# yanivw12/gs2mesh

Hardware: AMD Instinct MI355X
Metric: stereo-pair renders/sec + TSDF Mvoxel-updates/sec (higher is better)
Workload: dtype f32

## Files before the change

gs2mesh_amd/_lib.py:

```python
from __future__ import annotations

import ctypes as C

import numpy as np
import os

_HERE = os.path.dirname(os.path.abspath(__file__))
LIB_PATH = os.path.join(_HERE, "libgs2mesh_amd.so")

vp = C.c_void_p
i32 = C.c_int
i64 = C.c_int64
f32 = C.c_float
f64 = C.c_double


class Camera(C.Structure):
    _fields_ = [("width", C.c_int32), ("height", C.c_int32), ("tanfovx", f32), ("tanfovy", f32),
                ("viewmatrix", f32 * 16), ("projmatrix", f32 * 16), ("campos", f32 * 3)]


class Gaussians(C.Structure):
    _fields_ = [("P", C.c_int32), ("sh_degree", C.c_int32), ("M", C.c_int32), ("raw", C.c_int32),
                ("xyz", vp), ("scales", vp), ("rotations", vp), ("opacities", vp), ("shs", vp), ("shs_rest", vp)]
# ... 7 lines not shown
OPT_BIN_WORKGROUPS = 9
OPT_BIN_WG_THREADS = 10
OPT_BLEND_MODE = 11
TSDF_MAP_HEADER_BYTES = 32
OPT_BLEND_PROFILE = 12
OPT_BIN_LANE_TILES = 13
OPT_PROJECT_SHARED_READ = 14
BLEND_PROF_COUNTERS = ("waves", "wave_cycles", "dma_wait", "staging", "prefetch_issue", "loop", "epilogue", "batches",
                       "staged_instances", "listed_instances")
XFORM_SUM_F32, XFORM_RAW_F32, XFORM_SUM_PACKED = 0, 1, 2
XFORM_PACKED_MAX_FRAMES = 1023
OPT_DEBUG_SYNC = 3
OPT_STAGE_TIMING = 4
RASTER_STAGES = ("project", "hist_colscan", "tile_scan", "scatter", "sort_tiles", "blend", "count_tiles")
TSDF_STAGES = ("tsdf_touch", "tsdf_integrate")

_PROTOS = {
    "gs2m_version": (i32, []),
    "gs2m_last_error": (C.c_char_p, []),
    "gs2m_raster_create": (i32, [C.POINTER(vp), i32]),
    "gs2m_raster_destroy": (i32, [vp]),
    "gs2m_raster_set_option": (i32, [vp, i32, i32]),
    "gs2m_raster_reserve": (i32, [vp, i32, i32, i32, i32, i64]),
    "gs2m_rasterize_forward": (i32, [vp, i32, i32, i32, vp, i32, i32, vp, vp, vp, vp, vp, f32, vp, vp, vp, vp, vp,
                                     f32, f32, i32, vp, vp, i32, vp]),
    "gs2m_mark_visible": (i32, [i32, vp, vp, vp, vp, vp]),
    "gs2m_render_views": (i32, [vp, C.POINTER(Gaussians), C.POINTER(Camera), i32, C.POINTER(f32), f32, vp, vp, vp,
                                vp]),
    "gs2m_raster_pack_sh": (i32, [vp, C.POINTER(Gaussians), vp]),
    "gs2m_raster_pack_model": (i32, [vp, C.POINTER(Gaussians), vp, vp]),
    "gs2m_raster_pack_invalidate": (i32, [vp]),
    "gs2m_raster_status": (i32, [vp, vp, i32, C.POINTER(i64), C.POINTER(i32), C.POINTER(i64)]),
    "gs2m_raster_stage_times": (i32, [vp, vp, C.POINTER(f64), C.POINTER(i64)]),
    "gs2m_raster_blend_cycles": (i32, [vp, vp, C.POINTER(C.c_uint64)]),
    "gs2m_raster_download_geometry": (i32, [vp, vp, i32, i32, vp, vp, vp, vp, vp, vp]),
    "gs2m_raster_download_binning": (i32, [vp, vp, i32, i64, vp, C.c_int32, vp]),
    "gs2m_tsdf_extract_count": (i32, [vp, vp, C.POINTER(i64)]),
    "gs2m_tsdf_extract": (i32, [vp, vp, i64, vp, vp, C.POINTER(i64)]),
    "gs2m_tsdf_extract_indexed": (i32, [vp, vp, i64, vp, vp, vp, C.POINTER(i64)]),
    "gs2m_stereo_depth_occlusion": (i32, [vp, vp, i32, i32, f64, f64, vp, vp, vp]),
    "gs2m_mask_preprocess": (i32, [i32, i32, i32, C.POINTER(vp), C.POINTER(vp), i32, i32, i32, i32, C.POINTER(vp), vp, vp]),
    "gs2m_tsdf_create": (i32, [C.POINTER(vp), f64, f64, i32, i32, i32, i64, i32]),
    "gs2m_tsdf_destroy": (i32, [vp]),
    "gs2m_tsdf_reset": (i32, [vp, vp]),
    "gs2m_tsdf_integrate": (i32, [vp, vp, vp, vp, i32, i32, f64, f64, f64, f64, C.POINTER(f64), f64, f64, f64, vp]),
    "gs2m_tsdf_integrate_batch": (i32, [vp, i32, C.POINTER(vp), C.POINTER(vp), C.POINTER(vp), i32, i32, f64, f64, f64, f64,
                                        C.POINTER(f64), f64, f64, f64, vp]),
    "gs2m_tsdf_set_stage_timing": (i32, [vp, i32]),
    "gs2m_tsdf_stage_times": (i32, [vp, vp, C.POINTER(f64), C.POINTER(i64)]),
# ... 118 lines not shown
```

gs2mesh_amd/csrc/raster_api.hip:

```cpp
#include <stdarg.h>
#include <stdio.h>
#include <stdlib.h>
#include <string.h>

#include <string>
#include <vector>

#include "../../include/gs2mesh_amd.h"
#include "raster_internal.h"
#include "roctx_ranges.h"

static thread_local std::string g_err;
void gs2m_set_error(const char* fmt, ...) {
    char buf[1024];
    va_list ap;
    va_start(ap, fmt);
    vsnprintf(buf, sizeof(buf), fmt, ap);
    va_end(ap);
    g_err = buf;
}
extern "C" const char* gs2m_last_error(void) { return g_err.c_str(); }
extern "C" int gs2m_version(void) { return GS2M_VERSION; }

#define HIPCHK(expr)                                                                          \
    do {                                                                                      \
        hipError_t e__ = (expr);                                                              \
        if (e__ != hipSuccess) {                                                              \
            gs2m_set_error("%s failed: %s (%s:%d)", #expr, hipGetErrorString(e__), __FILE__, __LINE__); \
            return 1;                                                                         \
        }                                                                                     \
    } while (0)

#define GS2M_SORT_CLASSES_API 3
#define GS2M_MAX_STATUS 64

struct gs2m_raster {
    int device = 0;
    int opt_exact_cull = 0, opt_blend = 4, opt_debug = 0, opt_timing = 0, opt_tile_rows = 1, opt_pair_batch = 0;
    int opt_bin_workgroups = 256, opt_bin_wg_threads = 1024, opt_blend_mode = 2;
    int opt_blend_profile = 0;
    int opt_project_shared = 0;
    int opt_bin_lane_tiles = 4;
    unsigned long long* d_blend_prof = nullptr;
    struct EvPair {
        int stage;
        hipEvent_t a, b;
    };
    std::vector<EvPair> ev_live;
    std::vector<hipEvent_t> ev_free;
// ... 3 lines not shown
    unsigned long long* d_tilemask = nullptr;
    float* d_shpack = nullptr;
    size_t shpack_cap = 0;
    const float* pack_src = nullptr;
    const float* pack_src_rest = nullptr;
    int pack_P = 0;
    float* d_pk_xyz = nullptr;
    float* d_pk_scales = nullptr;
    float* d_pk_rots = nullptr;
    float* d_pk_opac = nullptr;
    int* d_order = nullptr;
    int* d_rank = nullptr;
    size_t pk_cap3 = 0, pk_cap3s = 0, pk_cap4 = 0, pk_cap1 = 0, order_cap = 0, rank_cap = 0;
    const float* model_src[4] = {nullptr, nullptr, nullptr, nullptr};
    bool model_packed = false;
    bool hint_valid = false;
    bool last_packed = false;
    const int* run_rank = nullptr;
    size_t mask_cap = 0;
    unsigned* d_hist = nullptr;
    size_t hist_cap = 0;
    unsigned* d_tile_count = nullptr;
    unsigned* d_tile_start = nullptr;
    size_t tile_cap = 0;
    unsigned* d_sort_lists = nullptr;
    size_t sort_lists_cap = 0;
    unsigned long long* d_keys = nullptr;
    unsigned long long* d_tmp = nullptr;
    size_t keys_cap_total = 0;
    unsigned inst_cap = 0;
    ViewStatus* d_status = nullptr;
// ... 45 lines not shown
    (void)hipFree(r->d_shpack);
    (void)hipFree(r->d_pk_xyz);
    (void)hipFree(r->d_pk_scales);
    (void)hipFree(r->d_pk_rots);
    (void)hipFree(r->d_pk_opac);
    (void)hipFree(r->d_order);
    (void)hipFree(r->d_rank);
    (void)hipFree(r->d_hist);
    (void)hipFree(r->d_tile_count);
    (void)hipFree(r->d_tile_start);
    (void)hipFree(r->d_sort_lists);
    (void)hipFree(r->d_keys);
    (void)hipFree(r->d_tmp);
    (void)hipFree(r->d_status);
    (void)hipFree(r->d_blend_prof);
    (void)hipHostFree(r->h_status);
    for (auto& p : r->ev_live) {
        (void)hipEventDestroy(p.a);
        (void)hipEventDestroy(p.b);
    }
    for (auto e : r->ev_free) (void)hipEventDestroy(e);
    delete r;
    return 0;
}

extern "C" int gs2m_raster_set_option(gs2m_raster* r, int option, int value) {
    if (!r) {
        gs2m_set_error("null handle");
        return 1;
    }
// ... 153 lines not shown
    StageTimer(gs2m_raster* r_, hipStream_t st_, int stage_) : r(r_), st(st_), stage(stage_), range(kStageRange[stage_]) {
        if (r->opt_timing) {
            a = ev_get(r);
            b = ev_get(r);
            if (a) (void)hipEventRecord(a, st);
        }
    }
    ~StageTimer() {
        if (a && b) {
            (void)hipEventRecord(b, st);
            r->ev_live.push_back({stage, a, b});
        }
    }
};

static int run_views(gs2m_raster* r, const GaussIn& g, int nv, int pairs, int W, int H, float* out_color,
                     unsigned char* out_rgb8, int* out_radii, int status_slot, hipStream_t st, const CamUniform* host_cams) {
    const int nvt = nv * pairs;
    const int gx = (W + GS2M_TILE - 1) / GS2M_TILE, gy = (H + GS2M_TILE - 1) / GS2M_TILE;
    const int gys = (gy + r->opt_tile_rows - 1) / r->opt_tile_rows;
    const int tiles = gx * gys;
    int hint[3] = {-1, -1, -1};
    int interleave = 1;
    if (r->hint_valid && r->last_tiles == tiles && r->last_nv == nvt) {
        unsigned nr_max = 0;
        for (int c = 0; c < 3; ++c) {
            unsigned m = 0;
            for (int v = 0; v < nvt; ++v) {
                const unsigned x = r->h_status[1 + status_slot + v].n_class[c];
                m = x > m ? x : m;
            }
            hint[c] = m > 0x3fffffffu ? -1 : (int)m;
        }
        for (int v = 0; v < nvt; ++v) {
            const unsigned x = r->h_status[1 + status_slot + v].num_rendered;
            nr_max = x > nr_max ? x : nr_max;
        }
        if (nr_max > 0u && nr_max <= 0x3fffffffu) interleave = (size_t)nr_max >= (size_t)800 * (size_t)tiles;
    }
    int chunk, n_wg;
    geometry(r, g.P, &chunk, &n_wg, pairs);
    int wg_threads = (gs2m_count_threads(chunk, r->opt_bin_wg_threads) + 63) / 64 * 64;
    while (wg_threads > 64 && (gs2m_scatter_lds_bytes(nv, tiles, wg_threads) > 160 * 1024 || gs2m_count_lds_bytes(nv, tiles, wg_threads) > 160 * 1024))
        wg_threads = (wg_threads / 2 + 63) / 64 * 64;
    const size_t lds = gs2m_scatter_lds_bytes(nv, tiles, wg_threads);
    const size_t lds_p = gs2m_count_lds_bytes(nv, tiles, wg_threads);
    if (lds > 160 * 1024 || lds_p > 160 * 1024) {
        gs2m_set_error("image %dx%d: %d views x %d tiles do not fit the 160 KiB LDS tile cursors", W, H, nv, tiles);
        return 1;
    }
    if (r->inst_cap == 0) {
        int64_t guess = (int64_t)g.P * 4;
// ... 21 lines not shown
        gs2m_launch_hist_colscan(st, nvt, r->d_hist, n_wg, tiles, r->d_tile_count);
    }
    if (dbg_check(r, st, "hist_colscan")) return 1;
    {
        StageTimer tm(r, st, GS2M_STAGE_TILESCAN);
        gs2m_launch_tile_scan(st, nvt, r->d_tile_count, r->d_tile_start, tiles, gx, r->h_status + 1 + status_slot, r->d_status, cap, r->d_sort_lists);
    }
    if (dbg_check(r, st, "tile_scan")) return 1;
    {
        StageTimer tm(r, st, GS2M_STAGE_SCATTER);
        if (gs2m_launch_scatter(nv, pairs, n_wg, wg_threads, lds, st, recs, g.P, r->d_cams, chunk, r->d_hist, r->d_tile_start,
                                r->d_tilemask, r->d_keys, cap, cull_arg_s, g.ids, g.ids != nullptr, r->opt_bin_lane_tiles))
            return 1;
    }
    if (dbg_check(r, st, "scatter")) return 1;
    {
        StageTimer tm(r, st, GS2M_STAGE_SORT);
        gs2m_launch_sort_tiles(st, nvt, r->d_keys, r->d_tmp, r->d_tile_start, tiles, cap, r->d_sort_lists, hint);
    }
    if (dbg_check(r, st, "sort_tiles")) return 1;
    {
        StageTimer tm(r, st, GS2M_STAGE_BLEND);
        if (gs2m_launch_blend(st, r->opt_blend, r->opt_tile_rows, nvt, gx, gy, r->d_keys, r->d_tile_start, recs, r->d_cams,
                              g.P, cap, out_color, out_rgb8, g.ids ? r->run_rank : nullptr,
                              r->d_sort_lists + (size_t)nvt * GS2M_SORT_CLASSES_API * (tiles + 1), r->opt_blend_mode,
                              r->opt_blend_profile ? r->d_blend_prof : nullptr, interleave))
            return 1;
    }
    if (dbg_check(r, st, "blend")) return 1;
    r->last_P = g.P;
    r->hint_valid = true;
    r->last_packed = g.ids != nullptr;
    r->last_nv = nvt;
    r->last_tiles = tiles;
    r->last_cap = cap;
    return 0;
}

extern "C" int gs2m_rasterize_forward(gs2m_raster* r, int P, int D, int M, const float* background, int width,
                                      int height, const float* means3D, const float* shs,
                                      const float* colors_precomp, const float* opacities, const float* scales,
                                      float scale_modifier, const float* rotations, const float* cov3D_precomp,
                                      const float* viewmatrix, const float* projmatrix, const float* cam_pos,
                                      float tan_fovx, float tan_fovy, int prefiltered, float* out_color,
                                      int* radii, int debug, gs2m_stream stream) {
    (void)prefiltered;
    if (!r) {
        gs2m_set_error("null handle");
        return 1;
    }
// ... 161 lines not shown
            u.gy = (H + GS2M_TILE - 1) / GS2M_TILE;
            u.bg[0] = bg[0];
            u.bg[1] = bg[1];
            u.bg[2] = bg[2];
            u.th = 16 * r->opt_tile_rows;
        }
        if (run_views(r, g, nv, pairs, W, H, out_color ? out_color + 3 * img * v0 : nullptr,
                      out_rgb8 ? out_rgb8 + 3 * img * v0 : nullptr,
                      out_radii ? out_radii + (size_t)gs->P * v0 : nullptr, v0, st, cu))
            return 1;
        v0 += nvt;
    }
    return 0;
}

static int pack_common(gs2m_raster* r, const gs2m_gaussians* gs, const int32_t* order, gs2m_stream stream, const char* who) {
    if (!r || !gs) {
        gs2m_set_error("%s: NULL argument", who);
        return 1;
    }
    r->pack_src = nullptr;
    r->pack_src_rest = nullptr;
    r->pack_P = 0;
    r->model_packed = false;
    if (gs->P <= 0 || gs->M != 16 || !gs->shs) return 0;
    HIPCHK(hipSetDevice(r->device));
    hipStream_t st = (hipStream_t)stream;
    const size_t P = (size_t)gs->P;
    const size_t groups = (P + 63) / 64;
    if (ensure(&r->d_shpack, &r->shpack_cap, groups * 12 * 64 * 4)) return 1;
// ... 227 lines not shown
```

gs2mesh_amd/csrc/raster_bin.hip:

```cpp
#include "raster_sort.h"
#include "raster_internal.h"

void gs2m_launch_hist_colscan(hipStream_t st, int nv, unsigned* hist, int n_wg, int tiles, unsigned* tile_count) {
    GS2M_LAUNCH(k_hist_colscan, dim3((tiles + 63) / 64, nv), dim3(64 * GS2M_COLSCAN_SEGS), 0, st, hist, n_wg, tiles, tile_count);
}
void gs2m_launch_tile_scan(hipStream_t st, int nv, const unsigned* tile_count, unsigned* tile_start, int tiles, int gx,
                           ViewStatus* status, ViewStatus* sticky, unsigned cap, unsigned* sort_lists) {
    GS2M_LAUNCH(k_tile_scan, dim3(nv), dim3(1024), 0, st, tile_count, tile_start, tiles, gx, status, sticky, cap, sort_lists);
}
size_t gs2m_sort_lists_words(int nv, int tiles) { return (size_t)nv * (GS2M_SORT_CLASSES * (tiles + 1) + tiles); }
void gs2m_launch_sort_tiles(hipStream_t st, int nv, unsigned long long* keys, unsigned long long* tmp,
                            const unsigned* tile_start, int tiles, unsigned cap, const unsigned* sort_lists, const int* class_hint) {
    const int fold = class_hint && class_hint[0] == 0 && class_hint[1] == 0 && class_hint[2] == 0;
    GS2M_LAUNCH(k_sort_tiles_small<4>, dim3((tiles + 3) / 4, nv), dim3(256), 0, st, keys, tile_start, tiles, cap, tmp, sort_lists, fold);
    if (fold) return;
    const int full[3] = {tiles < 1024 ? tiles : 1024, tiles < 512 ? tiles : 512, tiles < 512 ? tiles : 512};
    int g[3];
    for (int c = 0; c < 3; ++c) {
        g[c] = full[c];
        if (class_hint && class_hint[c] >= 0) {
            const int want = class_hint[c] + class_hint[c] / 2 + 16;
            g[c] = want < full[c] ? want : full[c];
        }
        if (g[c] < 1) g[c] = 1;
    }
    GS2M_LAUNCH(k_sort_tiles_bucket_4096x8, dim3(g[0], nv), dim3(512), 0, st, keys, tile_start, tiles, cap, sort_lists);
    GS2M_LAUNCH(k_sort_tiles_bucket_8192x8, dim3(g[1], nv), dim3(1024), 0, st, keys, tile_start, tiles, cap, sort_lists);
    GS2M_LAUNCH(k_sort_tiles, dim3(g[2], nv), dim3(256), 0, st, keys, tmp, tile_start, tiles, cap, sort_lists);
}
```

gs2mesh_amd/csrc/raster_internal.h:

```cpp
#pragma once
#include "raster_common.h"

size_t gs2m_scatter_lds_bytes(int nv, int tiles, int threads);
void gs2m_launch_project(int nv, int pairs, hipStream_t st, const GaussIn& g, CamUniform* cams, GeomRecs recs, int* radii,
                         int exact_cull, const CamUniform* host_cams, int shared_read);
int gs2m_launch_count_tiles(int nv, int pairs, int n_wg, int threads, size_t lds_bytes, hipStream_t st, GeomRecs recs, int P,
                            const CamUniform* cams, int chunk, unsigned* hist, unsigned long long* tilemask,
                            int exact_cull, int interleave, int lane_tiles);
int gs2m_count_threads(int chunk, int max_threads);
size_t gs2m_count_lds_bytes(int nv, int tiles, int threads);
int gs2m_launch_scatter(int nv, int pairs, int n_wg, int threads, size_t lds_bytes, hipStream_t st, GeomRecs recs, int P,
                        const CamUniform* cams, int chunk, const unsigned* hist, const unsigned* tile_start,
                        const unsigned long long* tilemask, unsigned long long* keys, unsigned cap, int exact_cull,
                        const int* ids, int interleave, int lane_tiles);
void gs2m_launch_pack_sh(hipStream_t st, int P, const float* shs, const float* shs_rest, float* packed, const int* order);
void gs2m_launch_pack_model(hipStream_t st, int P, const int* order, const float* xyz, const float* scales, const float* rots,
                            const float* opac, float* p_xyz, float* p_scales, float* p_rots, float* p_opac, int* rank,
                            unsigned* bad);
void gs2m_launch_mark_visible(hipStream_t st, int P, const float* xyz, const float* viewmatrix,
                              unsigned char* present);
void gs2m_launch_pack_camera(hipStream_t st, CamUniform* cams, int slot, const float* viewmatrix,
                             const float* projmatrix, const float* campos, const float* bg, float tanfovx,
                             float tanfovy, int W, int H, int th);

void gs2m_launch_hist_colscan(hipStream_t st, int nv, unsigned* hist, int n_wg, int tiles, unsigned* tile_count);
void gs2m_launch_tile_scan(hipStream_t st, int nv, const unsigned* tile_count, unsigned* tile_start, int tiles, int gx,
                           ViewStatus* status, ViewStatus* sticky, unsigned cap, unsigned* sort_lists);
size_t gs2m_sort_lists_words(int nv, int tiles);
void gs2m_launch_sort_tiles(hipStream_t st, int nv, unsigned long long* keys, unsigned long long* tmp,
                            const unsigned* tile_start, int tiles, unsigned cap, const unsigned* sort_lists, const int* class_hint);
int gs2m_launch_blend(hipStream_t st, int variant, int tile_rows, int nv, int gx, int gy, const unsigned long long* keys,
                      const unsigned* tile_start, GeomRecs recs, const CamUniform* cams, int P,
                      unsigned cap, float* out_color, unsigned char* out_rgb8, const int* rank, const unsigned* order,
                      int mode, unsigned long long* prof, int interleave_views);

void gs2m_set_error(const char* fmt, ...);
```

gs2mesh_amd/csrc/tsdf_api.hip:

```cpp
#include <math.h>
#include <stdio.h>
#include <string.h>

#include <mutex>
#include <vector>

#include "../../include/gs2mesh_amd.h"
#include "tsdf_common.h"
#include "tsdf_internal.h"
#include "roctx_ranges.h"

#define HIPCHK(expr)                                                                          \
    do {                                                                                      \
        hipError_t e__ = (expr);                                                              \
        if (e__ != hipSuccess) {                                                              \
            gs2m_set_error("%s failed: %s (%s:%d)", #expr, hipGetErrorString(e__), __FILE__, __LINE__); \
            return 1;                                                                         \
        }                                                                                     \
    } while (0)

struct gs2m_tsdf {
    int device = 0;
    double voxel_length = 0, sdf_trunc = 0, unit_length = 0;
    int color_type = 1, resolution = 16, stride = 4;
// ... 14 lines not shown
    char* mesh_scratch = nullptr;
    size_t mesh_scratch_cap = 0;
    int timing = 0;
    struct EvPair {
        int stage;
        hipEvent_t a, b;
        int frames;
    };
    std::vector<EvPair> ev_live;
    std::vector<hipEvent_t> ev_free;
    TsdfBatchFrame* d_bframes = nullptr;
    static const int kRing = 8;
    TsdfBatchFrame* h_bframes = nullptr;
    hipEvent_t ring_done[8] = {nullptr, nullptr, nullptr, nullptr, nullptr, nullptr, nullptr, nullptr};
    unsigned ring_next = 0;
};

static hipEvent_t tsdf_ev_get(gs2m_tsdf* t) {
    if (!t->ev_free.empty()) {
        hipEvent_t e = t->ev_free.back();
        t->ev_free.pop_back();
        return e;
    }
    hipEvent_t e;
    if (hipEventCreate(&e) != hipSuccess) return nullptr;
    return e;
}

static bool invert4x4(const double* m, double* inv) {
    double a[16];
// ... 17 lines not shown
    if (det == 0) return false;
    det = 1.0 / det;
    for (int i = 0; i < 16; i++) inv[i] = a[i] * det;
    return true;
}

static int zero_state(gs2m_tsdf* t, hipStream_t st, bool whole_pool, long long keep_first = -1) {
    TsdfVolume& V = t->V;
    if (whole_pool) {
        HIPCHK(hipMemsetAsync(V.tsdf, 0, sizeof(float) * (size_t)V.max_blocks * GS2M_TSDF_VOX, st));
        HIPCHK(hipMemsetAsync(V.weight, 0, sizeof(float) * (size_t)V.max_blocks * GS2M_TSDF_VOX, st));
        if (V.rgb) HIPCHK(hipMemsetAsync(V.rgb, 0, sizeof(unsigned) * 3 * (size_t)V.max_blocks * GS2M_TSDF_VOX, st));
        HIPCHK(hipMemsetAsync(V.halo, 0, (size_t)V.max_blocks, st));
    } else if (keep_first < 0) {
        gs2m_launch_tsdf_clear_used(st, V);
    } else {
        gs2m_launch_tsdf_clear_from(st, V, (unsigned)keep_first);
    }
    HIPCHK(hipMemsetAsync(V.hash_keys, 0xff, sizeof(unsigned long long) * (size_t)V.hash_cap, st));
    HIPCHK(hipMemsetAsync(V.hash_vals, 0xff, sizeof(int) * (size_t)V.hash_cap, st));
    HIPCHK(hipMemsetAsync(V.stamp, 0, sizeof(unsigned) * (size_t)V.hash_cap, st));
    HIPCHK(hipMemsetAsync(V.fmask, 0, sizeof(unsigned long long) * (size_t)V.hash_cap, st));
    HIPCHK(hipMemsetAsync(V.counters, 0, sizeof(unsigned) * 4, st));
    HIPCHK(hipMemsetAsync(V.totals, 0, sizeof(unsigned long long), st));
    return 0;
}

extern "C" int gs2m_tsdf_create(gs2m_tsdf** out, double voxel_length, double sdf_trunc, int color_type,
                                int volume_unit_resolution, int depth_sampling_stride, int64_t max_blocks,
                                int device) {
// ... 188 lines not shown
    if (fill_frame(t, f, width, height, fx, fy, cx, cy, extrinsic_w2c, depth_scale, depth_trunc, min_depth, mask != nullptr))
        return 1;
    HIPCHK(hipMemsetAsync(t->V.counters + 1, 0, sizeof(unsigned), st));
    hipEvent_t e0 = nullptr, e1 = nullptr, e2 = nullptr, e3 = nullptr;
    if (t->timing) {
        e0 = tsdf_ev_get(t);
        e1 = tsdf_ev_get(t);
        e2 = tsdf_ev_get(t);
        e3 = tsdf_ev_get(t);
    }
    const bool tm = e0 && e1 && e2 && e3;
    if (tm) (void)hipEventRecord(e0, st);
    {
        Gs2mRange rg("gs2m:tsdf_touch");
        gs2m_launch_tsdf_touch(st, t->V, f, depth, mask);
    }
    if (tm) {
        (void)hipEventRecord(e1, st);
        (void)hipEventRecord(e2, st);
    }
    {
        Gs2mRange rg("gs2m:tsdf_integrate");
        gs2m_launch_tsdf_integrate(st, t->n_cu * 7, t->V, f, depth, color, mask);
    }
    if (tm) {
        (void)hipEventRecord(e3, st);
        t->ev_live.push_back({0, e0, e1, 1});
        t->ev_live.push_back({1, e2, e3, 1});
    }
    return 0;
// ... 41 lines not shown
        HIPCHK(hipEventRecord(t->ring_done[slot], st));
        HIPCHK(hipMemsetAsync(t->V.counters + 1, 0, sizeof(unsigned), st));
        HIPCHK(hipMemsetAsync(t->V.counters + 3, 0, sizeof(unsigned), st));
        hipEvent_t e0 = nullptr, e1 = nullptr, e2 = nullptr, e3 = nullptr;
        if (t->timing) {
            e0 = tsdf_ev_get(t);
            e1 = tsdf_ev_get(t);
            e2 = tsdf_ev_get(t);
            e3 = tsdf_ev_get(t);
        }
        const bool tm = e0 && e1 && e2 && e3;
        if (tm) (void)hipEventRecord(e0, st);
        {
            Gs2mRange rg("gs2m:tsdf_touch_batch");
            gs2m_launch_tsdf_touch_batch(st, t->V, hb[0].f, nf, t->d_bframes);
        }
        if (tm) {
            (void)hipEventRecord(e1, st);
            (void)hipEventRecord(e2, st);
        }
        {
            Gs2mRange rg("gs2m:tsdf_integrate_batch");
            gs2m_launch_tsdf_integrate_batch(st, t->n_cu, t->V, t->d_bframes);
        }
        if (tm) {
            (void)hipEventRecord(e3, st);
            t->ev_live.push_back({0, e0, e1, nf});
            t->ev_live.push_back({1, e2, e3, nf});
        }
    }
    return 0;
}

extern "C" int gs2m_tsdf_set_stage_timing(gs2m_tsdf* t, int enable) {
    if (!t) {
        gs2m_set_error("null handle");
        return 1;
    }
    t->timing = enable != 0;
    return 0;
}

extern "C" int gs2m_tsdf_stage_times(gs2m_tsdf* t, gs2m_stream stream, double* total_ms, int64_t* launches) {
    if (!t || !total_ms || !launches) {
        gs2m_set_error("gs2m_tsdf_stage_times: NULL argument");
// ... 515 lines not shown
```

gs2mesh_amd/integration.py:

```python
from __future__ import annotations

import ctypes as C
import enum

import numpy as np

from . import _lib
from .rasterizer import _is_torch, _ptr, _stream_of

try:
    import torch
except Exception:
    torch = None


class TSDFVolumeColorType(enum.IntEnum):
    NoColor = 0
    RGB8 = 1
    Gray32 = 2


class PinholeCameraIntrinsic:
    def __init__(self, width, height, fx, fy, cx, cy):
        self.width, self.height = int(width), int(height)
# ... 37 lines not shown
    def __init__(self, voxel_length, sdf_trunc, color_type=TSDFVolumeColorType.RGB8, volume_unit_resolution=16,
                 depth_sampling_stride=4, max_blocks=32768, device=0, lib=None):
        self._lib = lib or _lib.get()
        if int(color_type) not in (0, 1):
            raise NotImplementedError("only NoColor / RGB8 volumes (tsdf_utils.py:56 uses RGB8)")
        self.voxel_length = float(voxel_length)
        self.sdf_trunc = float(sdf_trunc)
        self.color_type = TSDFVolumeColorType(int(color_type))
        self.max_blocks = int(max_blocks)
        self.device = device
        h = C.c_void_p()
        _lib.check(self._lib.gs2m_tsdf_create(C.byref(h), self.voxel_length, self.sdf_trunc, int(color_type),
                                              int(volume_unit_resolution), int(depth_sampling_stride),
                                              self.max_blocks, int(device)), self._lib)
        self._h = h
        self._keep = []
        self.frames_base = 0
        self.frames_injected = 0
        self.frames_local = 0
        self.replicated = False
        self.has_halo = False
        self.exchange_window = ((-32, -32, -32), (64, 64, 64))
        self._xbuf = {}

    def close(self):
        if getattr(self, "_h", None):
            self._lib.gs2m_tsdf_destroy(self._h)
            self._h = None

    def __del__(self):
        try:
            self.close()
        except Exception:
            pass

    def reset(self, stream=None):
        _lib.check(self._lib.gs2m_tsdf_reset(self._h, stream or C.c_void_p(0)), self._lib)
        self._reset_bookkeeping()

    def _reset_bookkeeping(self):
        self.frames_base = self.frames_local = self.frames_injected = 0
        self.replicated = False
        self.has_halo = False

    @property
    def frames_integrated(self):
        return self.frames_base + self.frames_injected + self.frames_local

    def exchange_buffer(self, name, shape, dtype, device):
# ... 217 lines not shown
```

gs2mesh_amd/pipeline.py:

```python
from __future__ import annotations

import numpy as np
import torch

from . import _lib
from .integration import PinholeCameraIntrinsic, RGBDImage, ScalableTSDFVolume
from .rasterizer import Rasterizer


class RenderFusePipeline:

    RASTER_OPTION_IDS = dict(exact_tile_cull=_lib.OPT_EXACT_TILE_CULL, tile_rows=_lib.OPT_TILE_ROWS,
                             blend_variant=_lib.OPT_BLEND_VARIANT, blend_mode=_lib.OPT_BLEND_MODE,
                             bin_workgroups=_lib.OPT_BIN_WORKGROUPS, bin_wg_threads=_lib.OPT_BIN_WG_THREADS,
                             bin_lane_tiles=_lib.OPT_BIN_LANE_TILES, project_shared_read=_lib.OPT_PROJECT_SHARED_READ)

    def __init__(self, gaussians: dict, width: int, height: int, volume: ScalableTSDFVolume | None = None,
                 intrinsic: PinholeCameraIntrinsic | None = None, inflight: int = 2, device: int = 0, *, fuse_batch=1,
                 pairs_per_launch: int = 1, spatial_order="auto", bg=(0.0, 0.0, 0.0), raster_options: dict | None = None):
        if inflight < 1:
            raise ValueError("inflight must be >= 1")
        self.g = gaussians
        if spatial_order == "auto":
            from .rasterizer import auto_spatial_order
# ... 63 lines not shown

    def prepare(self, cams, headroom: float = 1.3):
        first = None
        order = None
        for j, r in enumerate(self.rasterizers):
            if self.spatial_order:
                order = r.pack_model(self.g, order=order)
            else:
                r.pack_sh(self.g)
            res = r.render_views(self.g, cams, bg=self.bg, out_color=self.color[j][:2], out_rgb8=self.rgb8[j][:2],
                                 want_radii=(j == 0))
            r.reserve(int(self.g["xyz"].shape[0]), 2 * self.ppl, self.W, self.H, int(max(res["num_rendered"]) * headroom))
            if self.ppl > 1:
                r.render_views(self.g, list(cams) * self.ppl, bg=self.bg, out_color=self.color[j], out_rgb8=self._own8[j],
                               sync=False)
            if j == 0:
                first = res
        torch.cuda.synchronize(self.device)
        return first

    def model_updated(self):
        for r in self.rasterizers:
            r.invalidate_pack()
        self._model_seen = [False] * self.inflight

    def submit(self, cams, depth=None, extrinsic=None, depth_scale=1.0, depth_trunc=float("inf"), min_depth=0.0,
               mask=None):
        if self.ppl > 1:
            if depth is None:
                raise ValueError("pairs_per_launch > 1: every view is fused (depth required)")
# ... 186 lines not shown
```

gs2mesh_amd/rasterizer.py:

```python
from __future__ import annotations

import ctypes as C
import math

import numpy as np

from . import _lib

try:
    import torch
except Exception:
    torch = None


def _is_torch(x):
    return torch is not None and isinstance(x, torch.Tensor)


def _ptr(x, dtype=None, name="tensor"):
    return _lib.MEMORY.ptr(x, dtype, name)


_NP2T = {}
if torch is not None:
# ... 115 lines not shown
                                                C.byref(req)), self._lib)
        return list(nr)[:n_views], bool(ov.value), int(req.value)

    def stage_times(self, stream=None):
        n = len(_lib.RASTER_STAGES)
        ms = (C.c_double * n)()
        cnt = (C.c_int64 * n)()
        _lib.check(self._lib.gs2m_raster_stage_times(self._h, stream or C.c_void_p(0), ms, cnt), self._lib)
        return {name: (ms[i], cnt[i]) for i, name in enumerate(_lib.RASTER_STAGES)}

    def blend_cycles(self, stream=None):
        n = len(_lib.BLEND_PROF_COUNTERS)
        c = (C.c_uint64 * n)()
        _lib.check(self._lib.gs2m_raster_blend_cycles(self._h, stream or C.c_void_p(0), c), self._lib)
        return {name: int(c[i]) for i, name in enumerate(_lib.BLEND_PROF_COUNTERS)}

    def forward(self, means3D, opacities, viewmatrix, projmatrix, campos, bg, W, H, tanfovx, tanfovy, shs=None,
                colors_precomp=None, scales=None, rotations=None, cov3D_precomp=None, sh_degree=3,
                scale_modifier=1.0, prefiltered=False, debug=False, stream=None, sync=True):
        P = int(means3D.shape[0])
        D = int(sh_degree)
        M = 0 if shs is None or (hasattr(shs, "numel") and shs.numel() == 0) or getattr(shs, "size", 1) == 0 \
            else int(shs.shape[1])
        out = _empty(means3D, (3, int(H), int(W)), np.float32)
        radii = _empty(means3D, (P,), np.int32)
        st = _stream_of(means3D, stream)
        f32 = torch.float32 if _is_torch(means3D) else None

        def call():
            _lib.check(self._lib.gs2m_rasterize_forward(
# ... 118 lines not shown
```

include/gs2mesh_amd.h:

```cpp
#ifndef GS2MESH_AMD_H
#define GS2MESH_AMD_H

#include <stddef.h>
#include <stdint.h>

#ifdef __cplusplus
extern "C" {
#endif

#define GS2M_VERSION 600

typedef void* gs2m_stream;


int gs2m_version(void);
const char* gs2m_last_error(void);


typedef struct gs2m_raster gs2m_raster;

enum {
    GS2M_OPT_EXACT_TILE_CULL = 1,
    GS2M_OPT_BLEND_VARIANT = 2,
    GS2M_OPT_DEBUG_SYNC = 3,
// ... 63 lines not shown

int gs2m_raster_pack_model(gs2m_raster* r, const gs2m_gaussians* g, const int32_t* order ,
                           gs2m_stream stream);

int gs2m_raster_pack_invalidate(gs2m_raster* r);

int gs2m_raster_status(gs2m_raster* r, gs2m_stream stream, int n_views,
                       int64_t* num_rendered, int* overflow, int64_t* required);

int gs2m_raster_stage_times(gs2m_raster* r, gs2m_stream stream, double* total_ms,
                            int64_t* launches);

#define GS2M_BLEND_PROF_COUNTERS 10
int gs2m_raster_blend_cycles(gs2m_raster* r, gs2m_stream stream, uint64_t* counters);

int gs2m_raster_download_geometry(gs2m_raster* r, gs2m_stream stream, int v, int P,
                                  float* means2D, float* depths, float* conic_opacity,
                                  float* rgb, uint16_t* rect, uint32_t* tiles_touched);
int gs2m_raster_download_binning(gs2m_raster* r, gs2m_stream stream, int v, int64_t n,
                                 uint32_t* point_list, int32_t n_tiles, uint32_t* ranges);


typedef struct gs2m_tsdf gs2m_tsdf;

enum { GS2M_TSDF_COLOR_NONE = 0, GS2M_TSDF_COLOR_RGB8 = 1 };

int gs2m_tsdf_create(gs2m_tsdf** out, double voxel_length, double sdf_trunc, int color_type,
                     int volume_unit_resolution, int depth_sampling_stride, int64_t max_blocks,
                     int device);
int gs2m_tsdf_destroy(gs2m_tsdf* t);
int gs2m_tsdf_reset(gs2m_tsdf* t, gs2m_stream stream);

int gs2m_tsdf_integrate(gs2m_tsdf* t, const float* depth, const uint8_t* color,
                        const uint8_t* mask, int width, int height, double fx, double fy,
                        double cx, double cy, const double* extrinsic_w2c, double depth_scale,
                        double depth_trunc, double min_depth, gs2m_stream stream);

int gs2m_tsdf_integrate_batch(gs2m_tsdf* t, int n_frames, const float* const* depth, const uint8_t* const* color,
                              const uint8_t* const* mask, int width, int height, double fx, double fy, double cx,
                              double cy, const double* extrinsics_w2c, double depth_scale, double depth_trunc,
                              double min_depth, gs2m_stream stream);

int gs2m_tsdf_set_stage_timing(gs2m_tsdf* t, int enable);
int gs2m_tsdf_stage_times(gs2m_tsdf* t, gs2m_stream stream, double* total_ms, int64_t* launches);

int gs2m_tsdf_status(gs2m_tsdf* t, gs2m_stream stream, int64_t* n_blocks,
                     int64_t* block_updates, int* overflow);

int gs2m_tsdf_flags_device(gs2m_tsdf* t, uint32_t* flags_dev, gs2m_stream stream);

int gs2m_tsdf_download(gs2m_tsdf* t, gs2m_stream stream, int64_t n, int32_t* keys,
                       float* tsdf, float* weight, uint32_t* rgb_sum);

int gs2m_tsdf_block_keys(gs2m_tsdf* t, int64_t n, int32_t* keys, gs2m_stream stream);

int gs2m_tsdf_pack_sum(gs2m_tsdf* t, const int32_t* keys, int64_t n, float* buf, gs2m_stream stream);
// ... 53 lines not shown
```

Baseline: 4111.

## Add per-shape sort hint cache and warm-up passes for raster and TSDF kernels

Replaces the single last-pass sort-class hint with a small LRU cache of hints keyed by tile count and view count. Alternating pass shapes (different pair counts) can then each reuse their own class-size hints instead of falling back to the unhinted sort path. Adds warm-up entry points that launch every raster and TSDF kernel variant once on dummy data at setup, so first-launch costs (code object loading, lazy init) are paid outside the timed loop. Also adds launch counters and last-pass introspection for diagnostics.

Result: no change. 4114, median of 6 (+0.1%).

```diff
diff --git a/gs2mesh_amd/_lib.py b/gs2mesh_amd/_lib.py
--- a/gs2mesh_amd/_lib.py
+++ b/gs2mesh_amd/_lib.py
@@ -45,6 +45,10 @@
 OPT_STAGE_TIMING = 4
 RASTER_STAGES = ("project", "hist_colscan", "tile_scan", "scatter", "sort_tiles", "blend", "count_tiles")
 TSDF_STAGES = ("tsdf_touch", "tsdf_integrate")
+PASS_INFO = ("hint_class0", "hint_class1", "hint_class2", "interleave", "class_kernels", "views", "tiles")
+RASTER_KERNELS = ("project", "count_tiles", "hist_colscan", "tile_scan", "scatter", "sort_small", "sort_class0", "sort_class1",
+                  "sort_class2", "blend_m2_views", "blend_m2_interleaved", "blend_m3_views", "blend_m3_interleaved", "blend_other")
+TSDF_KERNELS = ("touch_batch", "compact", "integrate_batch", "clear_fmask", "clear_used")
 
 _PROTOS = {
     "gs2m_version": (i32, []),
@@ -64,6 +68,11 @@
     "gs2m_raster_status": (i32, [vp, vp, i32, C.POINTER(i64), C.POINTER(i32), C.POINTER(i64)]),
     "gs2m_raster_stage_times": (i32, [vp, vp, C.POINTER(f64), C.POINTER(i64)]),
     "gs2m_raster_blend_cycles": (i32, [vp, vp, C.POINTER(C.c_uint64)]),
+    "gs2m_raster_warm": (i32, [vp, i32, i32, i32, i32, vp]),
+    "gs2m_raster_last_pass": (i32, [vp, C.POINTER(C.c_int32)]),
+    "gs2m_raster_launch_counts": (i32, [vp, C.POINTER(i64)]),
+    "gs2m_tsdf_warm": (i32, [vp, vp]),
+    "gs2m_tsdf_launch_counts": (i32, [vp, C.POINTER(i64)]),
     "gs2m_raster_download_geometry": (i32, [vp, vp, i32, i32, vp, vp, vp, vp, vp, vp]),
     "gs2m_raster_download_binning": (i32, [vp, vp, i32, i64, vp, C.c_int32, vp]),
     "gs2m_tsdf_extract_count": (i32, [vp, vp, C.POINTER(i64)]),
diff --git a/gs2mesh_amd/csrc/raster_api.hip b/gs2mesh_amd/csrc/raster_api.hip
--- a/gs2mesh_amd/csrc/raster_api.hip
+++ b/gs2mesh_amd/csrc/raster_api.hip
@@ -33,6 +33,8 @@
 
 #define GS2M_SORT_CLASSES_API 3
 #define GS2M_MAX_STATUS 64
+#define GS2M_HINT_SHAPES 4
+#define GS2M_WARM_P 256
 
 struct gs2m_raster {
     int device = 0;
@@ -66,7 +68,20 @@
     size_t pk_cap3 = 0, pk_cap3s = 0, pk_cap4 = 0, pk_cap1 = 0, order_cap = 0, rank_cap = 0;
     const float* model_src[4] = {nullptr, nullptr, nullptr, nullptr};
     bool model_packed = false;
+    struct ShapeHint {
+        int tiles = 0, nvt = 0;
+        unsigned n_class[GS2M_SORT_CLASSES_API] = {0, 0, 0};
+        unsigned nr_max = 0;
+        unsigned long long used = 0;
+    };
+    ShapeHint hints[GS2M_HINT_SHAPES];
+    unsigned long long pass_no = 0;
     bool hint_valid = false;
+    int last_slot = 0;
+    int last_info[GS2M_PASS_INFO_WORDS] = {-1, -1, -1, 1, 0, 0, 0};
+    int64_t launches[GS2M_RASTER_KERNELS] = {};
+    float* d_warm = nullptr;
+    int* d_warm_ids = nullptr;
     bool last_packed = false;
     const int* run_rank = nullptr;
     size_t mask_cap = 0;
@@ -142,6 +157,8 @@
     (void)hipFree(r->d_tmp);
     (void)hipFree(r->d_status);
     (void)hipFree(r->d_blend_prof);
+    (void)hipFree(r->d_warm);
+    (void)hipFree(r->d_warm_ids);
     (void)hipHostFree(r->h_status);
     for (auto& p : r->ev_live) {
         (void)hipEventDestroy(p.a);
@@ -325,28 +342,52 @@
     }
 };
 
+static gs2m_raster::ShapeHint* hint_find(gs2m_raster* r, int tiles, int nvt) {
+    for (auto& e : r->hints)
+        if (e.nvt == nvt && e.tiles == tiles) {
+            e.used = r->pass_no;
+            return &e;
+        }
+    return nullptr;
+}
+static void hint_refresh(gs2m_raster* r, int tiles, int nvt, int slot) {
+    gs2m_raster::ShapeHint* e = hint_find(r, tiles, nvt);
+    if (!e) {
+        e = &r->hints[0];
+        for (auto& x : r->hints)
+            if (x.nvt == 0 || (e->nvt != 0 && x.used < e->used)) e = &x;
+        e->tiles = tiles;
+        e->nvt = nvt;
+    }
+    e->used = r->pass_no;
+    e->nr_max = 0;
+    for (int c = 0; c < GS2M_SORT_CLASSES_API; ++c) e->n_class[c] = 0;
+    for (int v = 0; v < nvt; ++v) {
+        const ViewStatus& s = r->h_status[1 + slot + v];
+        for (int c = 0; c < GS2M_SORT_CLASSES_API; ++c) e->n_class[c] = s.n_class[c] > e->n_class[c] ? s.n_class[c] : e->n_class[c];
+        e->nr_max = s.num_rendered > e->nr_max ? s.num_rendered : e->nr_max;
+    }
+}
+
 static int run_views(gs2m_raster* r, const GaussIn& g, int nv, int pairs, int W, int H, float* out_color,
-                     unsigned char* out_rgb8, int* out_radii, int status_slot, hipStream_t st, const CamUniform* host_cams) {
+                     unsigned char* out_rgb8, int* out_radii, int status_slot, hipStream_t st, const CamUniform* host_cams,
+                     bool warm = false) {
     const int nvt = nv * pairs;
     const int gx = (W + GS2M_TILE - 1) / GS2M_TILE, gy = (H + GS2M_TILE - 1) / GS2M_TILE;
     const int gys = (gy + r->opt_tile_rows - 1) / r->opt_tile_rows;
     const int tiles = gx * gys;
     int hint[3] = {-1, -1, -1};
     int interleave = 1;
-    if (r->hint_valid && r->last_tiles == tiles && r->last_nv == nvt) {
-        unsigned nr_max = 0;
-        for (int c = 0; c < 3; ++c) {
-            unsigned m = 0;
-            for (int v = 0; v < nvt; ++v) {
-                const unsigned x = r->h_status[1 + status_slot + v].n_class[c];
-                m = x > m ? x : m;
-            }
-            hint[c] = m > 0x3fffffffu ? -1 : (int)m;
-        }
-        for (int v = 0; v < nvt; ++v) {
-            const unsigned x = r->h_status[1 + status_slot + v].num_rendered;
-            nr_max = x > nr_max ? x : nr_max;
-        }
+    ++r->pass_no;
+    if (!warm && r->hint_valid) {
+        hint_refresh(r, r->last_tiles, r->last_nv, r->last_slot);
+        if (r->last_tiles == tiles && r->last_nv == nvt && r->last_slot != status_slot) hint_refresh(r, tiles, nvt, status_slot);
+    }
+    if (warm) {
+        hint[0] = hint[1] = hint[2] = 1;
+    } else if (const gs2m_raster::ShapeHint* e = hint_find(r, tiles, nvt)) {
+        const unsigned nr_max = e->nr_max;
+        for (int c = 0; c < 3; ++c) hint[c] = e->n_class[c] > 0x3fffffffu ? -1 : (int)e->n_class[c];
         if (nr_max > 0u && nr_max <= 0x3fffffffu) interleave = (size_t)nr_max >= (size_t)800 * (size_t)tiles;
     }
     int chunk, n_wg;
@@ -398,26 +439,45 @@
             return 1;
     }
     if (dbg_check(r, st, "scatter")) return 1;
+    int n_class_kernels = 0;
     {
         StageTimer tm(r, st, GS2M_STAGE_SORT);
-        gs2m_launch_sort_tiles(st, nvt, r->d_keys, r->d_tmp, r->d_tile_start, tiles, cap, r->d_sort_lists, hint);
+        n_class_kernels = gs2m_launch_sort_tiles(st, nvt, r->d_keys, r->d_tmp, r->d_tile_start, tiles, cap, r->d_sort_lists, hint);
     }
     if (dbg_check(r, st, "sort_tiles")) return 1;
-    {
+    r->launches[GS2M_RK_PROJECT] += g.P > 0;
+    r->launches[GS2M_RK_COUNT_TILES]++;
+    r->launches[GS2M_RK_HIST_COLSCAN]++;
+    r->launches[GS2M_RK_TILE_SCAN]++;
+    r->launches[GS2M_RK_SCATTER]++;
+    r->launches[GS2M_RK_SORT_SMALL]++;
+    for (int c = 0; c < n_class_kernels; ++c) r->launches[GS2M_RK_SORT_CLASS0 + c]++;
+    const bool forms = warm && r->opt_blend == 4 && r->opt_blend_mode >= 2 && !r->opt_blend_profile;
+    for (int k = 0; k < (forms ? 4 : 1); ++k) {
+        const int mode = forms ? 2 + (k >> 1) : r->opt_blend_mode, il = forms ? (k & 1) : interleave;
         StageTimer tm(r, st, GS2M_STAGE_BLEND);
         if (gs2m_launch_blend(st, r->opt_blend, r->opt_tile_rows, nvt, gx, gy, r->d_keys, r->d_tile_start, recs, r->d_cams,
                               g.P, cap, out_color, out_rgb8, g.ids ? r->run_rank : nullptr,
-                              r->d_sort_lists + (size_t)nvt * GS2M_SORT_CLASSES_API * (tiles + 1), r->opt_blend_mode,
-                              r->opt_blend_profile ? r->d_blend_prof : nullptr, interleave))
+                              r->d_sort_lists + (size_t)nvt * GS2M_SORT_CLASSES_API * (tiles + 1), mode,
+                              r->opt_blend_profile ? r->d_blend_prof : nullptr, il))
             return 1;
+        const bool m23 = r->opt_blend == 4 && mode >= 2 && !r->opt_blend_profile;
+        r->launches[!m23 ? GS2M_RK_BLEND_OTHER : GS2M_RK_BLEND_M2_VIEWS + 2 * (mode - 2) + (il && nvt > 1 ? 1 : 0)]++;
     }
     if (dbg_check(r, st, "blend")) return 1;
+    if (warm) return 0;
     r->last_P = g.P;
     r->hint_valid = true;
     r->last_packed = g.ids != nullptr;
     r->last_nv = nvt;
     r->last_tiles = tiles;
     r->last_cap = cap;
+    r->last_slot = status_slot;
+    for (int c = 0; c < 3; ++c) r->last_info[c] = hint[c];
+    r->last_info[3] = interleave;
+    r->last_info[4] = n_class_kernels;
+    r->last_info[5] = nvt;
+    r->last_info[6] = tiles;
     return 0;
 }
 
@@ -609,6 +669,75 @@
     return 0;
 }
 
+extern "C" int gs2m_raster_warm(gs2m_raster* r, int nv, int pairs, int W, int H, gs2m_stream stream) {
+    if (!r) {
+        gs2m_set_error("null handle");
+        return 1;
+    }
+    if (nv < 1 || nv > GS2M_MAX_VIEWS || pairs < 1 || pairs > GS2M_MAX_PAIRS || W <= 0 || H <= 0) {
+        gs2m_set_error("gs2m_raster_warm: %d views x %d groups of %d x %d pixels is not a launch shape", nv, pairs, W, H);
+        return 1;
+    }
+    hipStream_t st = (hipStream_t)stream;
+    HIPCHK(hipSetDevice(r->device));
+    int per = GS2M_MAX_VIEWS;
+    while (per > 1 && gs2m_scatter_lds_bytes(per, binning_tiles(r, W, H), 64) > 160 * 1024) per--;
+    if (nv > per) nv = per;
+    if (per != GS2M_MAX_VIEWS) pairs = 1;
+    const size_t words = (size_t)GS2M_WARM_P * 48;
+    if (!r->d_warm) {
+        HIPCHK(hipMalloc((void**)&r->d_warm, words * sizeof(float)));
+        HIPCHK(hipMalloc((void**)&r->d_warm_ids, (GS2M_WARM_P + 1) * sizeof(int)));
+        HIPCHK(hipMemsetAsync(r->d_warm, 0, words * sizeof(float), st));
+        HIPCHK(hipMemsetAsync(r->d_warm_ids, 0, (GS2M_WARM_P + 1) * sizeof(int), st));
+    }
+    GaussIn g;
+    g.xyz = g.scales = g.rots = g.opac = g.shs = r->d_warm;
+    g.shs_rest = nullptr;
+    g.shs_packed = r->pack_src ? r->d_warm : nullptr;
+    g.cov3D_precomp = nullptr;
+    g.colors_precomp = nullptr;
+    g.ids = r->model_packed ? r->d_warm_ids : nullptr;
+    g.P = GS2M_WARM_P;
+    g.D = 3;
+    g.M = 16;
+    g.raw = 1;
+    g.scale_modifier = 1.0f;
+    CamUniform cu[GS2M_MAX_PASS_VIEWS];
+    memset(cu, 0, sizeof(cu));
+    for (int k = 0; k < nv * pairs; ++k) {
+        cu[k].W = W;
+        cu[k].H = H;
+        cu[k].gx = (W + GS2M_TILE - 1) / GS2M_TILE;
+        cu[k].gy = (H + GS2M_TILE - 1) / GS2M_TILE;
+        cu[k].tanfovx = cu[k].tanfovy = cu[k].focal_x = cu[k].focal_y = 1.0f;
+        cu[k].th = 16 * r->opt_tile_rows;
+    }
+    const int* saved_rank = r->run_rank;
+    r->run_rank = r->d_warm_ids;
+    const int rc = run_views(r, g, nv, pairs, W, H, nullptr, nullptr, nullptr, GS2M_MAX_STATUS - nv * pairs, st, cu, true);
+    r->run_rank = saved_rank;
+    return rc;
+}
+
+extern "C" int gs2m_raster_last_pass(gs2m_raster* r, int32_t* info) {
+    if (!r || !info) {
+        gs2m_set_error("gs2m_raster_last_pass: NULL argument");
+        return 1;
+    }
+    for (int i = 0; i < GS2M_PASS_INFO_WORDS; ++i) info[i] = r->last_info[i];
+    return 0;
+}
+
+extern "C" int gs2m_raster_launch_counts(gs2m_raster* r, int64_t* counts) {
+    if (!r || !counts) {
+        gs2m_set_error("gs2m_raster_launch_counts: NULL argument");
+        return 1;
+    }
+    for (int i = 0; i < GS2M_RASTER_KERNELS; ++i) counts[i] = r->launches[i];
+    return 0;
+}
+
 static int pack_common(gs2m_raster* r, const gs2m_gaussians* gs, const int32_t* order, gs2m_stream stream, const char* who) {
     if (!r || !gs) {
         gs2m_set_error("%s: NULL argument", who);
diff --git a/gs2mesh_amd/csrc/raster_bin.hip b/gs2mesh_amd/csrc/raster_bin.hip
--- a/gs2mesh_amd/csrc/raster_bin.hip
+++ b/gs2mesh_amd/csrc/raster_bin.hip
@@ -9,11 +9,11 @@
     GS2M_LAUNCH(k_tile_scan, dim3(nv), dim3(1024), 0, st, tile_count, tile_start, tiles, gx, status, sticky, cap, sort_lists);
 }
 size_t gs2m_sort_lists_words(int nv, int tiles) { return (size_t)nv * (GS2M_SORT_CLASSES * (tiles + 1) + tiles); }
-void gs2m_launch_sort_tiles(hipStream_t st, int nv, unsigned long long* keys, unsigned long long* tmp,
+int gs2m_launch_sort_tiles(hipStream_t st, int nv, unsigned long long* keys, unsigned long long* tmp,
                             const unsigned* tile_start, int tiles, unsigned cap, const unsigned* sort_lists, const int* class_hint) {
     const int fold = class_hint && class_hint[0] == 0 && class_hint[1] == 0 && class_hint[2] == 0;
     GS2M_LAUNCH(k_sort_tiles_small<4>, dim3((tiles + 3) / 4, nv), dim3(256), 0, st, keys, tile_start, tiles, cap, tmp, sort_lists, fold);
-    if (fold) return;
+    if (fold) return 0;
     const int full[3] = {tiles < 1024 ? tiles : 1024, tiles < 512 ? tiles : 512, tiles < 512 ? tiles : 512};
     int g[3];
     for (int c = 0; c < 3; ++c) {
@@ -27,4 +27,5 @@
     GS2M_LAUNCH(k_sort_tiles_bucket_4096x8, dim3(g[0], nv), dim3(512), 0, st, keys, tile_start, tiles, cap, sort_lists);
     GS2M_LAUNCH(k_sort_tiles_bucket_8192x8, dim3(g[1], nv), dim3(1024), 0, st, keys, tile_start, tiles, cap, sort_lists);
     GS2M_LAUNCH(k_sort_tiles, dim3(g[2], nv), dim3(256), 0, st, keys, tmp, tile_start, tiles, cap, sort_lists);
+    return GS2M_SORT_CLASSES;
 }
diff --git a/gs2mesh_amd/csrc/raster_internal.h b/gs2mesh_amd/csrc/raster_internal.h
--- a/gs2mesh_amd/csrc/raster_internal.h
+++ b/gs2mesh_amd/csrc/raster_internal.h
@@ -27,7 +27,7 @@
 void gs2m_launch_tile_scan(hipStream_t st, int nv, const unsigned* tile_count, unsigned* tile_start, int tiles, int gx,
                            ViewStatus* status, ViewStatus* sticky, unsigned cap, unsigned* sort_lists);
 size_t gs2m_sort_lists_words(int nv, int tiles);
-void gs2m_launch_sort_tiles(hipStream_t st, int nv, unsigned long long* keys, unsigned long long* tmp,
+int gs2m_launch_sort_tiles(hipStream_t st, int nv, unsigned long long* keys, unsigned long long* tmp,
                             const unsigned* tile_start, int tiles, unsigned cap, const unsigned* sort_lists, const int* class_hint);
 int gs2m_launch_blend(hipStream_t st, int variant, int tile_rows, int nv, int gx, int gy, const unsigned long long* keys,
                       const unsigned* tile_start, GeomRecs recs, const CamUniform* cams, int P,
diff --git a/gs2mesh_amd/csrc/tsdf_api.hip b/gs2mesh_amd/csrc/tsdf_api.hip
--- a/gs2mesh_amd/csrc/tsdf_api.hip
+++ b/gs2mesh_amd/csrc/tsdf_api.hip
@@ -52,6 +52,7 @@
     TsdfBatchFrame* h_bframes = nullptr;
     hipEvent_t ring_done[8] = {nullptr, nullptr, nullptr, nullptr, nullptr, nullptr, nullptr, nullptr};
     unsigned ring_next = 0;
+    int64_t launches[GS2M_TSDF_KERNELS] = {0, 0, 0, 0, 0};
 };
 
 static hipEvent_t tsdf_ev_get(gs2m_tsdf* t) {
@@ -99,6 +100,7 @@
         HIPCHK(hipMemsetAsync(V.halo, 0, (size_t)V.max_blocks, st));
     } else if (keep_first < 0) {
         gs2m_launch_tsdf_clear_used(st, V);
+        t->launches[4]++;
     } else {
         gs2m_launch_tsdf_clear_from(st, V, (unsigned)keep_first);
     }
@@ -317,6 +319,7 @@
     {
         Gs2mRange rg("gs2m:tsdf_touch");
         gs2m_launch_tsdf_touch(st, t->V, f, depth, mask);
+        t->launches[1]++;
     }
     if (tm) {
         (void)hipEventRecord(e1, st);
@@ -388,6 +391,8 @@
         {
             Gs2mRange rg("gs2m:tsdf_touch_batch");
             gs2m_launch_tsdf_touch_batch(st, t->V, hb[0].f, nf, t->d_bframes);
+            t->launches[0]++;
+            t->launches[1]++;
         }
         if (tm) {
             (void)hipEventRecord(e1, st);
@@ -396,6 +401,8 @@
         {
             Gs2mRange rg("gs2m:tsdf_integrate_batch");
             gs2m_launch_tsdf_integrate_batch(st, t->n_cu, t->V, t->d_bframes);
+            t->launches[2]++;
+            t->launches[3]++;
         }
         if (tm) {
             (void)hipEventRecord(e3, st);
@@ -403,6 +410,38 @@
             t->ev_live.push_back({1, e2, e3, nf});
         }
     }
+    return 0;
+}
+
+extern "C" int gs2m_tsdf_warm(gs2m_tsdf* t, gs2m_stream stream) {
+    if (!t) {
+        gs2m_set_error("null handle");
+        return 1;
+    }
+    HIPCHK(hipSetDevice(t->device));
+    hipStream_t st = (hipStream_t)stream;
+    HIPCHK(hipMemsetAsync(t->d_bframes, 0, sizeof(TsdfBatchFrame), st));
+    HIPCHK(hipMemsetAsync(t->V.counters + 1, 0, sizeof(unsigned), st));
+    HIPCHK(hipMemsetAsync(t->V.counters + 3, 0, sizeof(unsigned), st));
+    TsdfFrame f;
+    memset(&f, 0, sizeof(f));
+    f.nx = 1;
+    f.ny = 1;
+    gs2m_launch_tsdf_touch_batch(st, t->V, f, 1, t->d_bframes);
+    gs2m_launch_tsdf_integrate_batch(st, t->n_cu, t->V, t->d_bframes);
+    TsdfVolume none = t->V;
+    none.max_blocks = 0;
+    gs2m_launch_tsdf_clear_used(st, none);
+    for (int i = 0; i < GS2M_TSDF_KERNELS; ++i) t->launches[i]++;
+    return 0;
+}
+
+extern "C" int gs2m_tsdf_launch_counts(gs2m_tsdf* t, int64_t* counts) {
+    if (!t || !counts) {
+        gs2m_set_error("gs2m_tsdf_launch_counts: NULL argument");
+        return 1;
+    }
+    for (int i = 0; i < GS2M_TSDF_KERNELS; ++i) counts[i] = t->launches[i];
     return 0;
 }
 
diff --git a/gs2mesh_amd/integration.py b/gs2mesh_amd/integration.py
--- a/gs2mesh_amd/integration.py
+++ b/gs2mesh_amd/integration.py
@@ -75,6 +75,7 @@
                                               int(volume_unit_resolution), int(depth_sampling_stride),
                                               self.max_blocks, int(device)), self._lib)
         self._h = h
+        _lib.check(self._lib.gs2m_tsdf_warm(self._h, C.c_void_p(0)), self._lib)
         self._keep = []
         self.frames_base = 0
         self.frames_injected = 0
@@ -94,6 +95,11 @@
             self.close()
         except Exception:
             pass
+
+    def launch_counts(self):
+        c = (C.c_int64 * len(_lib.TSDF_KERNELS))()
+        _lib.check(self._lib.gs2m_tsdf_launch_counts(self._h, c), self._lib)
+        return {name: int(c[i]) for i, name in enumerate(_lib.TSDF_KERNELS)}
 
     def reset(self, stream=None):
         _lib.check(self._lib.gs2m_tsdf_reset(self._h, stream or C.c_void_p(0)), self._lib)
diff --git a/gs2mesh_amd/pipeline.py b/gs2mesh_amd/pipeline.py
--- a/gs2mesh_amd/pipeline.py
+++ b/gs2mesh_amd/pipeline.py
@@ -101,6 +101,8 @@
             if self.ppl > 1:
                 r.render_views(self.g, list(cams) * self.ppl, bg=self.bg, out_color=self.color[j], out_rgb8=self._own8[j],
                                sync=False)
+            for pairs in range(1, self.ppl + 1):
+                r.warm(2, pairs, self.W, self.H)
             if j == 0:
                 first = res
         torch.cuda.synchronize(self.device)
diff --git a/gs2mesh_amd/rasterizer.py b/gs2mesh_amd/rasterizer.py
--- a/gs2mesh_amd/rasterizer.py
+++ b/gs2mesh_amd/rasterizer.py
@@ -153,6 +153,20 @@
         c = (C.c_uint64 * n)()
         _lib.check(self._lib.gs2m_raster_blend_cycles(self._h, stream or C.c_void_p(0), c), self._lib)
         return {name: int(c[i]) for i, name in enumerate(_lib.BLEND_PROF_COUNTERS)}
+
+    def warm(self, n_views, pairs, W, H, stream=None):
+        st = stream if stream is not None else _lib.MEMORY.current_stream(self.device)
+        _lib.check(self._lib.gs2m_raster_warm(self._h, int(n_views), int(pairs), int(W), int(H), st), self._lib)
+
+    def last_pass(self):
+        info = (C.c_int32 * len(_lib.PASS_INFO))()
+        _lib.check(self._lib.gs2m_raster_last_pass(self._h, info), self._lib)
+        return {name: int(info[i]) for i, name in enumerate(_lib.PASS_INFO)}
+
+    def launch_counts(self):
+        c = (C.c_int64 * len(_lib.RASTER_KERNELS))()
+        _lib.check(self._lib.gs2m_raster_launch_counts(self._h, c), self._lib)
+        return {name: int(c[i]) for i, name in enumerate(_lib.RASTER_KERNELS)}
 
     def forward(self, means3D, opacities, viewmatrix, projmatrix, campos, bg, W, H, tanfovx, tanfovy, shs=None,
                 colors_precomp=None, scales=None, rotations=None, cov3D_precomp=None, sh_degree=3,
diff --git a/include/gs2mesh_amd.h b/include/gs2mesh_amd.h
--- a/include/gs2mesh_amd.h
+++ b/include/gs2mesh_amd.h
@@ -101,6 +101,28 @@
 #define GS2M_BLEND_PROF_COUNTERS 10
 int gs2m_raster_blend_cycles(gs2m_raster* r, gs2m_stream stream, uint64_t* counters);
 
+int gs2m_raster_warm(gs2m_raster* r, int nv, int pairs, int W, int H, gs2m_stream stream);
+
+#define GS2M_PASS_INFO_WORDS 7
+int gs2m_raster_last_pass(gs2m_raster* r, int32_t* info);
+
+enum {
+    GS2M_RK_PROJECT = 0,
+    GS2M_RK_COUNT_TILES = 1,
+    GS2M_RK_HIST_COLSCAN = 2,
+    GS2M_RK_TILE_SCAN = 3,
+    GS2M_RK_SCATTER = 4,
+    GS2M_RK_SORT_SMALL = 5,
+    GS2M_RK_SORT_CLASS0 = 6,
+    GS2M_RK_BLEND_M2_VIEWS = 9,
+    GS2M_RK_BLEND_M2_INTERLEAVED = 10,
+    GS2M_RK_BLEND_M3_VIEWS = 11,
+    GS2M_RK_BLEND_M3_INTERLEAVED = 12,
+    GS2M_RK_BLEND_OTHER = 13,
+    GS2M_RASTER_KERNELS = 14
+};
+int gs2m_raster_launch_counts(gs2m_raster* r, int64_t* counts);
+
 int gs2m_raster_download_geometry(gs2m_raster* r, gs2m_stream stream, int v, int P,
                                   float* means2D, float* depths, float* conic_opacity,
                                   float* rgb, uint16_t* rect, uint32_t* tiles_touched);
@@ -127,6 +149,10 @@
                               const uint8_t* const* mask, int width, int height, double fx, double fy, double cx,
                               double cy, const double* extrinsics_w2c, double depth_scale, double depth_trunc,
                               double min_depth, gs2m_stream stream);
+
+#define GS2M_TSDF_KERNELS 5
+int gs2m_tsdf_warm(gs2m_tsdf* t, gs2m_stream stream);
+int gs2m_tsdf_launch_counts(gs2m_tsdf* t, int64_t* counts);
 
 int gs2m_tsdf_set_stage_timing(gs2m_tsdf* t, int enable);
 int gs2m_tsdf_stage_times(gs2m_tsdf* t, gs2m_stream stream, double* total_ms, int64_t* launches);
```
